# unibas-gravis/GiNGR

Hardware: AMD Instinct MI355X
Metric: GiNGR update iters/sec, 50k<->50k CPD (higher is better)
Workload: dtype f64; 1 GPU; CPD update, synthetic Gaussian clouds 50000<->50000, GPMM rank 100, w=0.1, rigid global transform, sigma2_0=5032.781; points=50000, targets=50000, rank=100, parallelism=row-shard x1, exchange=single shard

## Files before the change

gingr_amd/csrc/cpd_pairs.hip:

```cpp
#include "common.h"
#include "block_sum.h"
#include "box_device.h"
#include "cpd_plan.h"
#include "fastexp.h"

namespace {

constexpr int kBlock = 256;

constexpr int kTB = 11;
constexpr int kTabN = 1 << kTB;

#ifdef GINGR_STAMPS
__device__ unsigned long long *g_stamp_buf = nullptr;
constexpr int kStampWaves = 1 << 15;
struct Stamps {
    unsigned long long *p;
    long long c0;
    __device__ __forceinline__ void begin(int kernel) {
        const unsigned wg = blockIdx.y * gridDim.x + blockIdx.x;
        const unsigned w = wg * 4 + (threadIdx.x >> 6);
        p = (g_stamp_buf && w < kStampWaves) ? g_stamp_buf + ((size_t)kernel * kStampWaves + w) * 8 : nullptr;
        c0 = clock64();
        mark(0);
// ... 83 lines not shown
    unsigned long long act, slot[PT];
    const double *sub;
    const int32_t *bad;
    double negc;

    __device__ __forceinline__ void init(int64_t c0_, int64_t c1_, int q_, const double *sub_, const int32_t *bad_, double negc_) {
        c0 = c0_;
        c1 = c1_;
        q = q_;
        sub = sub_;
        bad = bad_;
        negc = negc_;
        t0 = c0 / kTile;
        nparts = c1 > c0 ? (int)((c1 - 1) / kTile - t0 + 1) : 0;
        pbase = 0;
        act = 0;
    }
    __device__ __forceinline__ void bounds(int p, int64_t *ib, int64_t *ie) const {
        const int64_t a = (t0 + p) * kTile, b = a + kTile;
        *ib = a > c0 ? a : c0;
        *ie = b < c1 ? b : c1;
    }
    __device__ __forceinline__ void batch(const Box &own, const Box (&sown)[PT]) {
        const int lane = threadIdx.x & 63;
        const int p = pbase + lane;
        int64_t ib, ie;
        bounds(p, &ib, &ie);
        const bool has = p < nparts && q * 64 < (int)(ie - ib);
        bool on = has;
        bool son[PT];
#pragma unroll
        for (int t = 0; t < PT; ++t) son[t] = has;
        if (has && sub && !(bad && bad[(t0 + p)])) {
            const double *qbox = sub + (ib / 64 + q) * 6;
            if (FINE) {
                on = false;
#pragma unroll
                for (int t = 0; t < PT; ++t) {
                    son[t] = !(box_gap2(sown[t], qbox) * negc > GINGR_CULL_SCALED(kTabN));
                    on = on || son[t];
                }
            } else {
                on = !(box_gap2(own, qbox) * negc > GINGR_CULL_SCALED(kTabN));
            }
        }
        act = __ballot(on);
        if (FINE) {
#pragma unroll
            for (int t = 0; t < PT; ++t) slot[t] = __ballot(son[t]);
        }
        pbase += 64;
    }
    __device__ __forceinline__ bool next(const Box &own, const Box (&sown)[PT], int64_t *ib, int64_t *ie, unsigned *mask) {
        while (act == 0) {
            if (pbase >= nparts) return false;
            batch(own, sown);
        }
        const int l = __builtin_ctzll(act);
        act &= act - 1;
        bounds(pbase - 64 + l, ib, ie);
        unsigned m = (1u << PT) - 1u;
        if (FINE) {
            m = 0;
#pragma unroll
            for (int t = 0; t < PT; ++t) m |= (unsigned)((slot[t] >> l) & 1ull) << t;
        }
        *mask = m;
        return true;
    }
};

__device__ __forceinline__ void fair_priority(int64_t done, int64_t total) {
    const int64_t f = total > 0 ? (4 * done) / total : 3;
    if (f <= 0)
        __builtin_amdgcn_s_setprio(3);
    else if (f == 1)
        __builtin_amdgcn_s_setprio(2);
    else if (f == 2)
        __builtin_amdgcn_s_setprio(1);
    else
        __builtin_amdgcn_s_setprio(0);
}

template <int PT, bool CLAMP, bool MASKED>
__device__ __forceinline__ void colsum_tile(const P4 *tile, int j0, int j1, unsigned mask, const double (&x)[PT],
                                            const double (&y)[PT], const double (&z)[PT], double (&acc)[PT], double c, double lim,
                                            const double *T) {
#pragma unroll 2
    for (int ii = j0; ii < j1; ++ii) {
        const P4 p = tile[ii];
#pragma unroll
        for (int t = 0; t < PT; ++t) {
            if (MASKED && !((mask >> t) & 1u)) continue;
            const double dx = x[t] - p.x, dy = y[t] - p.y, dz = z[t] - p.z;
            double d2 = __builtin_fma(dz, dz, __builtin_fma(dy, dy, dx * dx));
            if (CLAMP) d2 = fastexp_clamp_d2(d2, lim);
            acc[t] += fastexp2_floor_scaled(d2, c, T);
        }
    }
}

constexpr double kExpandTol = 1e-12;

__device__ __forceinline__ bool use_expansion(double rmax_centered, double c) {
    const double ratio = 3.0 * rmax_centered * rmax_centered * (-c) * (0.69314718055994530942 / kTabN);
    return ratio * 7.7e-16 < kExpandTol;
}

__device__ __forceinline__ double expand_owned_magic(double n, double *frac) {
    const double ni = __builtin_rint(n);
    *frac = n - ni;
    return GINGR_EXP_MAGIC8 + ni;
}
__device__ __forceinline__ double expand_owned_scale(double frac) { return exp2(frac * (1.0 / kTabN)); }

template <int PT, bool MASKED>
__device__ __forceinline__ void colsum_tile_expand(const P4 *tile, int j0, int j1, unsigned mask, const double (&x)[PT],
                                                   const double (&y)[PT], const double (&z)[PT], const double (&mg)[PT],
                                                   double (&acc)[PT], const double *T) {
#pragma unroll 2
    for (int ii = j0; ii < j1; ++ii) {
        const P4 p = tile[ii];
#pragma unroll
        for (int t = 0; t < PT; ++t) {
            if (MASKED && !((mask >> t) & 1u)) continue;
            const double A = __builtin_fma(z[t], p.z, __builtin_fma(y[t], p.y, __builtin_fma(x[t], p.x, p.w)));
            acc[t] += fastexp2_floor_core(A + mg[t], __builtin_amdgcn_fract(A), T);
        }
    }
}

template <int PT, bool FINE>
__global__ __launch_bounds__(kBlock) void cpd_colsum_kernel(Cloud fit, Cloud tgt, const double *__restrict__ sigma2,
                                                            const double *__restrict__ aux,
                                                            const double *__restrict__ fit_boxes, ChunkPlan plan,
                                                            double *__restrict__ partial, int32_t *regime_out) {
    __shared__ double T[kTabN];
    __shared__ P4 tile[kTile];
    __shared__ double sred[4][64 * PT];
    __shared__ double sfrac[64 * PT];
    STAMP_DECL
    STAMP_BEGIN(0)
    FloorTableRegs trom;
    fastexp_floor_table_fetch256(trom);
    const double s2in = sigma2[0], aux0 = aux[0], aux1 = aux[1], cx = aux[2], cy = aux[3], cz = aux[4];
    const int tid = threadIdx.x, lane = tid & 63;
    const int q = __builtin_amdgcn_readfirstlane(tid >> 6);
    const int64_t jbase = (int64_t)blockIdx.x * (64 * PT) + lane;
    double x[PT], y[PT], z[PT], n[PT], acc[PT];
    bool okv[PT];
#pragma unroll
    for (int t = 0; t < PT; ++t) {
        const int64_t j = jbase + (int64_t)t * 64;
        const bool ok = j < tgt.n;
        okv[t] = ok;
        x[t] = ok ? tgt.x[j] : 0.0;
        y[t] = ok ? tgt.y[j] : 0.0;
        z[t] = ok ? tgt.z[j] : 0.0;
    }
    int64_t i0, i1;
    plan.range(blockIdx.y, fit.n, &i0, &i1);
    const int q0 = q * 64;
    double lx = 0.0, ly = 0.0, lz = 0.0;
    const int64_t spec_ib = i0;
    {
        const int64_t e = min((i0 / kTile + 1) * kTile, i1), i = i0 + q0 + lane;
        if (i < e) {
            lx = fit.x[i];
            ly = fit.y[i];
            lz = fit.z[i];
        }
    }
    const double c = fastexp_scale_for_variance<kTB>(2.0 * s2in);
    const double am = aux0 + aux1;
    if (regime_out && blockIdx.x == 0 && blockIdx.y == 0 && threadIdx.x == 0) {
        *regime_out = (fit_boxes && 3.0 * am * am * (-c) > kFineCullRatio * GINGR_CULL_SCALED(kTabN)) ? 1 : 0;
        __threadfence_system();
    }
    const bool clamp = fastexp_needs_clamp(3.0 * am * am, c);
    const bool expand = use_expansion(fmax(aux0, aux1), c);
    const double lim = fastexp_d2_limit<kTB>(c);
    const double m2c = -2.0 * c;
    fastexp_floor_table_park256(T, trom);
    const Box own = wave_bbox<PT>(x, y, z, okv);
    constexpr unsigned kAllSlots = (1u << PT) - 1u;
    Box sown[PT];
    if (FINE) slot_boxes<PT>(x, y, z, okv, sown);
    const double *fit_sub = fit_boxes ? fit_boxes + ((fit.n + kTile - 1) / kTile) * 6 : nullptr;
#pragma unroll
    for (int t = 0; t < PT; ++t) {
        if (expand) {
            x[t] -= cx;
            y[t] -= cy;
            z[t] -= cz;
        }
        double fr;
        n[t] = expand_owned_magic(c * __builtin_fma(z[t], z[t], __builtin_fma(y[t], y[t], x[t] * x[t])), &fr);
        if (q == 0) sfrac[t * 64 + lane] = fr;
        acc[t] = 0.0;
    }
    STAMP(1)
    __syncthreads();
    STAMP(2)
    fastexp_round_down();
    struct Work {
        int64_t ib, ie;
        unsigned mask;
        bool valid;
    };
    PartWalk<PT, FINE> walk;
    walk.init(i0, i1, q, fit_boxes ? fit_sub : nullptr, nullptr, -c);
    auto find = [&]() {
        Work w{0, 0, kAllSlots, false};
        w.valid = walk.next(own, sown, &w.ib, &w.ie, &w.mask);
        return w;
    };
    auto issue = [&](const Work &w) {
        const int64_t i = w.ib + q0 + lane;
        if (i < w.ie) {
            lx = fit.x[i];
            ly = fit.y[i];
            lz = fit.z[i];
        }
    };
    Work cur = find();
    if (cur.valid && cur.ib != spec_ib) issue(cur);
#ifdef GINGR_STAMPS
    bool first__ = true;
#endif
    while (cur.valid) {
        if (plan.fair) fair_priority(cur.ib - i0, i1 - i0);
        __builtin_amdgcn_wave_barrier();
        if (cur.ib + q0 + lane < cur.ie) {
            if (expand) {
                const double fx = lx - cx, fy = ly - cy, fz = lz - cz;
                tile[q0 + lane] = P4{m2c * fx, m2c * fy, m2c * fz, c * __builtin_fma(fz, fz, __builtin_fma(fy, fy, fx * fx))};
            } else {
                tile[q0 + lane] = P4{lx, ly, lz, 0.0};
            }
        }
        __builtin_amdgcn_wave_barrier();
#ifdef GINGR_STAMPS
        if (first__) { STAMP(3) first__ = false; }
#endif
        const Work nxt = find();
        if (nxt.valid) issue(nxt);
        const int q1 = min((int)(cur.ie - cur.ib), q0 + 64);
        const unsigned mask = cur.mask;
        if (expand) {
            if (!FINE || mask == kAllSlots)
                colsum_tile_expand<PT, false>(tile, q0, q1, mask, x, y, z, n, acc, T);
            else
                colsum_tile_expand<PT, true>(tile, q0, q1, mask, x, y, z, n, acc, T);
        } else if (clamp) {
            if (!FINE || mask == kAllSlots)
                colsum_tile<PT, true, false>(tile, q0, q1, mask, x, y, z, acc, c, lim, T);
            else
                colsum_tile<PT, true, true>(tile, q0, q1, mask, x, y, z, acc, c, lim, T);
        } else {
            if (!FINE || mask == kAllSlots)
                colsum_tile<PT, false, false>(tile, q0, q1, mask, x, y, z, acc, c, lim, T);
            else
                colsum_tile<PT, false, true>(tile, q0, q1, mask, x, y, z, acc, c, lim, T);
        }
        cur = nxt;
    }
    fastexp_round_nearest();
    STAMP(4)
#pragma unroll
    for (int t = 0; t < PT; ++t) sred[q][t * 64 + lane] = acc[t];
    __syncthreads();
    for (int p = tid; p < 64 * PT; p += kBlock) {
        double v = (sred[0][p] + sred[1][p]) + (sred[2][p] + sred[3][p]);
        if (expand) v *= expand_owned_scale(sfrac[p]);
        const int64_t j = (int64_t)blockIdx.x * (64 * PT) + p;
        if (j < tgt.n) partial[(int64_t)blockIdx.y * tgt.n + j] = v;
    }
    STAMP_END
}

__global__ void chunk_reduce_kernel(const double *__restrict__ partial, int nchunks, int64_t n, double *__restrict__ out) {
    const int64_t j = (int64_t)blockIdx.x * blockDim.x + threadIdx.x;
    if (j >= n) return;
    double s = 0.0;
    for (int c = 0; c < nchunks; ++c) s += partial[(int64_t)c * n + j];
    out[j] = s;
}

constexpr int kScalarBlocks = 256;

__global__ __launch_bounds__(256) void cpd_den_finalize_kernel(Cloud tgt, const double *__restrict__ sigma2, double w,
                                                               double m_over_n, double *__restrict__ den,
                                                               double *__restrict__ inv_den, double *__restrict__ Pt1,
                                                               int32_t *__restrict__ tile_bad, double *__restrict__ part,
                                                               double *__restrict__ scalars,
                                                               const double *__restrict__ chunk_partial, int nchunks) {
    __shared__ double sh[256];
    const double s2 = sigma2[0];
    const double c = w / (1.0 - w) * pow(2.0 * 3.14159265358979323846 * s2, 1.5) * m_over_n;
    double xpx = 0.0;
    for (int64_t jt = (int64_t)blockIdx.x * 256; jt < tgt.n; jt += (int64_t)kScalarBlocks * 256) {
        const int64_t j = jt + threadIdx.x;
        int bad = 0;
        if (j < tgt.n) {
        double colsum;
        if (chunk_partial) {
            colsum = 0.0;
#pragma unroll 8
            for (int ch = 0; ch < nchunks; ++ch) colsum += chunk_partial[(int64_t)ch * tgt.n + j];
        } else {
            colsum = den[j];
        }
        const double d = colsum + c;
        const double inv = 1.0 / d;
        const double pt1 = colsum / d;
        den[j] = d;
        inv_den[j] = inv;
        Pt1[j] = pt1;
        bad = !(fabs(inv) <= 1.79769313486231570815e308);
        const double xx = tgt.x[j], yy = tgt.y[j], zz = tgt.z[j];
        xpx += pt1 * (xx * xx + yy * yy + zz * zz);
        }
        const int any_bad = __syncthreads_or(bad);
        if (tile_bad && threadIdx.x == 0) tile_bad[jt / kTile] = any_bad;
    }
    const double tot = block_sum<256>(xpx, sh);
    if (threadIdx.x == 0) {
        part[blockIdx.x] = tot;
        if (blockIdx.x == 0) scalars[5] = c;
    }
}

template <int PT, bool CLAMP, bool MASKED>
__device__ __forceinline__ void rowstats_tile(const P4 *tile, const P4 *tw, int j0, int j1, unsigned mask,
                                              const double (&x)[PT], const double (&y)[PT], const double (&z)[PT],
                                              double (&a1)[PT], double (&ax)[PT], double (&ay)[PT], double (&az)[PT], double c,
                                              double lim, const double *T) {
#pragma unroll 2
    for (int jj = j0; jj < j1; ++jj) {
        const P4 p = tile[jj];
        const P4 q = tw[jj];
#pragma unroll
        for (int t = 0; t < PT; ++t) {
            if (MASKED && !((mask >> t) & 1u)) continue;
            const double dx = p.x - x[t], dy = p.y - y[t], dz = p.z - z[t];
            double d2 = __builtin_fma(dz, dz, __builtin_fma(dy, dy, dx * dx));
            if (CLAMP) d2 = fastexp_clamp_d2(d2, lim);
            const double k = fastexp2_floor_scaled(d2, c, T);
            a1[t] = __builtin_fma(k, p.w, a1[t]);
            ax[t] = __builtin_fma(k, q.x, ax[t]);
            ay[t] = __builtin_fma(k, q.y, ay[t]);
            az[t] = __builtin_fma(k, q.z, az[t]);
        }
    }
}

template <int PT, bool MASKED>
__device__ __forceinline__ void rowstats_tile_expand(const P4 *tile, const P4 *tw, int j0, int j1, unsigned mask,
                                                     const double (&x)[PT], const double (&y)[PT], const double (&z)[PT],
                                                     const double (&mg)[PT], double (&a1)[PT], double (&ax)[PT], double (&ay)[PT],
                                                     double (&az)[PT], const double *T) {
#pragma unroll 2
    for (int jj = j0; jj < j1; ++jj) {
        const P4 p = tile[jj];
        const P4 q = tw[jj];
#pragma unroll
        for (int t = 0; t < PT; ++t) {
            if (MASKED && !((mask >> t) & 1u)) continue;
            const double A = __builtin_fma(z[t], p.z, __builtin_fma(y[t], p.y, __builtin_fma(x[t], p.x, p.w)));
            const double k = fastexp2_floor_core(A + mg[t], __builtin_amdgcn_fract(A), T);
            a1[t] = __builtin_fma(k, q.w, a1[t]);
            ax[t] = __builtin_fma(k, q.x, ax[t]);
            ay[t] = __builtin_fma(k, q.y, ay[t]);
            az[t] = __builtin_fma(k, q.z, az[t]);
        }
    }
}

template <int PT, bool FINE>
__global__ __launch_bounds__(kBlock, (PT >= 4 ? 3 : 4)) void cpd_rowstats_kernel(Cloud fit, Cloud tgt, const double *__restrict__ sigma2,
                                                              const double *__restrict__ aux,
                                                              const double *__restrict__ inv_den,
                                                              const double *__restrict__ tgt_boxes,
                                                              const int32_t *__restrict__ tile_bad, ChunkPlan plan,
                                                              double *__restrict__ partial, int32_t *regime_out) {
    constexpr int kRed = 4 * 4 * 64 * PT;
    constexpr int kLoop = kTabN + 4 * kTile + 4 * kTile;
    __shared__ double smem[kRed > kLoop ? kRed : kLoop];
    __shared__ double sfrac[64 * PT];
    double *T = smem;
    P4 *tile = reinterpret_cast<P4 *>(smem + kTabN);
    P4 *tw = reinterpret_cast<P4 *>(smem + kTabN + 4 * kTile);
    STAMP_DECL
    STAMP_BEGIN(1)
    FloorTableRegs trom;
    fastexp_floor_table_fetch256(trom);
    const double s2in = sigma2[0], aux0 = aux[0], aux1 = aux[1], cx = aux[2], cy = aux[3], cz = aux[4];
    const int tid = threadIdx.x, lane = tid & 63;
    const int q = __builtin_amdgcn_readfirstlane(tid >> 6);
    const int64_t ibase = (int64_t)blockIdx.x * (64 * PT) + lane;
    double x[PT], y[PT], z[PT], n[PT], a1[PT], ax[PT], ay[PT], az[PT];
    bool okv[PT];
#pragma unroll
    for (int t = 0; t < PT; ++t) {
        const int64_t i = ibase + (int64_t)t * 64;
        const bool ok = i < fit.n;
        okv[t] = ok;
        x[t] = ok ? fit.x[i] : 0.0;
        y[t] = ok ? fit.y[i] : 0.0;
        z[t] = ok ? fit.z[i] : 0.0;
    }
    int64_t j0, j1;
    plan.range(blockIdx.y, tgt.n, &j0, &j1);
    const int q0 = q * 64;
    double lx = 0.0, ly = 0.0, lz = 0.0, linv = 0.0;
    const int64_t spec_jb = j0;
    {
        const int64_t e = min((j0 / kTile + 1) * kTile, j1), j = j0 + q0 + lane;
        if (j < e) {
            lx = tgt.x[j];
            ly = tgt.y[j];
            lz = tgt.z[j];
            linv = inv_den[j];
        }
    }
    const double c = fastexp_scale_for_variance<kTB>(2.0 * s2in);
    const double am = aux0 + aux1;
    if (regime_out && blockIdx.x == 0 && blockIdx.y == 0 && threadIdx.x == 0) {
        *regime_out = (tgt_boxes && 3.0 * am * am * (-c) > kFineCullRatio * GINGR_CULL_SCALED(kTabN)) ? 1 : 0;
        __threadfence_system();
    }
    const bool clamp = fastexp_needs_clamp(3.0 * am * am, c);
    const bool expand = use_expansion(fmax(aux0, aux1), c);
    const double lim = fastexp_d2_limit<kTB>(c);
    const double m2c = -2.0 * c;
    fastexp_floor_table_park256(T, trom);
    const Box own = wave_bbox<PT>(x, y, z, okv);
    constexpr unsigned kAllSlots = (1u << PT) - 1u;
    Box sown[PT];
    if (FINE) slot_boxes<PT>(x, y, z, okv, sown);
    const double *tgt_sub = tgt_boxes ? tgt_boxes + ((tgt.n + kTile - 1) / kTile) * 6 : nullptr;
#pragma unroll
    for (int t = 0; t < PT; ++t) {
        if (expand) {
            x[t] -= cx;
            y[t] -= cy;
            z[t] -= cz;
        }
        double fr;
        n[t] = expand_owned_magic(c * __builtin_fma(z[t], z[t], __builtin_fma(y[t], y[t], x[t] * x[t])), &fr);
        if (q == 0) sfrac[t * 64 + lane] = fr;
        a1[t] = ax[t] = ay[t] = az[t] = 0.0;
    }
    STAMP(1)
    __syncthreads();
    STAMP(2)
    fastexp_round_down();
    struct Work {
        int64_t jb, je;
        unsigned mask;
        bool valid;
    };
    PartWalk<PT, FINE> walk;
    walk.init(j0, j1, q, tgt_boxes ? tgt_sub : nullptr, tgt_boxes ? tile_bad : nullptr, -c);
    auto find = [&]() {
        Work w{0, 0, kAllSlots, false};
        w.valid = walk.next(own, sown, &w.jb, &w.je, &w.mask);
        return w;
    };
    auto issue = [&](const Work &w) {
        const int64_t j = w.jb + q0 + lane;
        if (j < w.je) {
            lx = tgt.x[j];
            ly = tgt.y[j];
            lz = tgt.z[j];
            linv = inv_den[j];
        }
    };
    Work cur = find();
    if (cur.valid && cur.jb != spec_jb) issue(cur);
#ifdef GINGR_STAMPS
    bool first__ = true;
#endif
    while (cur.valid) {
        if (plan.fair) fair_priority(cur.jb - j0, j1 - j0);
        __builtin_amdgcn_wave_barrier();
        if (cur.jb + q0 + lane < cur.je) {
            const double inv = linv;
            if (expand) {
                const double tx = lx - cx, ty = ly - cy, tz = lz - cz;
                const double ax_ = m2c * tx, ay_ = m2c * ty, az_ = m2c * tz;
                tile[q0 + lane] = P4{ax_, ay_, az_, c * __builtin_fma(tz, tz, __builtin_fma(ty, ty, tx * tx))};
                tw[q0 + lane] = P4{ax_ * inv, ay_ * inv, az_ * inv, inv};
            } else {
                tile[q0 + lane] = P4{lx, ly, lz, inv};
                tw[q0 + lane] = P4{lx * inv, ly * inv, lz * inv, inv};
            }
        }
        __builtin_amdgcn_wave_barrier();
#ifdef GINGR_STAMPS
        if (first__) { STAMP(3) first__ = false; }
#endif
        const Work nxt = find();
        if (nxt.valid) issue(nxt);
        const int q1 = min((int)(cur.je - cur.jb), q0 + 64);
        const unsigned mask = cur.mask;
        if (expand) {
            if (!FINE || mask == kAllSlots)
                rowstats_tile_expand<PT, false>(tile, tw, q0, q1, mask, x, y, z, n, a1, ax, ay, az, T);
            else
                rowstats_tile_expand<PT, true>(tile, tw, q0, q1, mask, x, y, z, n, a1, ax, ay, az, T);
        } else if (clamp) {
            if (!FINE || mask == kAllSlots)
                rowstats_tile<PT, true, false>(tile, tw, q0, q1, mask, x, y, z, a1, ax, ay, az, c, lim, T);
            else
                rowstats_tile<PT, true, true>(tile, tw, q0, q1, mask, x, y, z, a1, ax, ay, az, c, lim, T);
        } else {
            if (!FINE || mask == kAllSlots)
                rowstats_tile<PT, false, false>(tile, tw, q0, q1, mask, x, y, z, a1, ax, ay, az, c, lim, T);
            else
                rowstats_tile<PT, false, true>(tile, tw, q0, q1, mask, x, y, z, a1, ax, ay, az, c, lim, T);
        }
        cur = nxt;
    }
    fastexp_round_nearest();
    STAMP(4)
    __syncthreads();
    constexpr int kPts = 64 * PT;
    double *sred = smem;
#pragma unroll
    for (int t = 0; t < PT; ++t) {
        sred[(q * 4 + 0) * kPts + t * 64 + lane] = a1[t];
        sred[(q * 4 + 1) * kPts + t * 64 + lane] = ax[t];
        sred[(q * 4 + 2) * kPts + t * 64 + lane] = ay[t];
        sred[(q * 4 + 3) * kPts + t * 64 + lane] = az[t];
    }
    __syncthreads();
    const int64_t M = fit.n;
    double *base = partial + (int64_t)blockIdx.y * 4 * M;
    const double back = expand ? -0.5 / c : 1.0;
    for (int p = tid; p < kPts; p += kBlock) {
        double v[4];
#pragma unroll
        for (int pl = 0; pl < 4; ++pl)
            v[pl] = (sred[(0 * 4 + pl) * kPts + p] + sred[(1 * 4 + pl) * kPts + p]) + (sred[(2 * 4 + pl) * kPts + p] + sred[(3 * 4 + pl) * kPts + p]);
        if (expand) {
            const double e = expand_owned_scale(sfrac[p]);
#pragma unroll
            for (int pl = 0; pl < 4; ++pl) v[pl] *= e;
        }
        const int64_t i = (int64_t)blockIdx.x * kPts + p;
        if (i < M) {
            base[i] = v[0];
            base[M + i] = expand ? __builtin_fma(cx, v[0], back * v[1]) : v[1];
            base[2 * M + i] = expand ? __builtin_fma(cy, v[0], back * v[2]) : v[2];
            base[3 * M + i] = expand ? __builtin_fma(cz, v[0], back * v[3]) : v[3];
        }
    }
    STAMP_END
}

template <int ROWS>
__global__ __launch_bounds__(4 * ROWS) void rowstats_reduce_kernel(const double *__restrict__ partial, int nchunks, Cloud fit,
                                                                   double *__restrict__ P1, double *__restrict__ PX,
                                                                   double *__restrict__ part, CpdObsArgs obs) {
    __shared__ double sh[ROWS];
    __shared__ double quart[3][4][ROWS];
    const int64_t M = fit.n;
    const int row = threadIdx.x % ROWS, g = threadIdx.x / ROWS;
    const int c0 = (int)((int64_t)g * nchunks / 4), c1 = (int)((int64_t)(g + 1) * nchunks / 4);
    double np = 0.0, tr = 0.0, ypy = 0.0;
    for (int64_t i0 = (int64_t)blockIdx.x * ROWS; i0 < M; i0 += (int64_t)kScalarBlocks * ROWS) {
        const int64_t i = i0 + row;
        const bool ok = i < M;
        double v[4] = {0.0, 0.0, 0.0, 0.0};
        double yx = 0.0, yy = 0.0, yz = 0.0, rf[3] = {0.0, 0.0, 0.0}, mn[3] = {0.0, 0.0, 0.0};
        int masked = 0;
        if (ok) {
            if (g == 0) {
                yx = fit.x[i];
                yy = fit.y[i];
                yz = fit.z[i];
                if (obs.weight) {
                    masked = obs.lm_mask ? obs.lm_mask[i] : 0;
#pragma unroll
                    for (int d = 0; d < 3; ++d) {
                        rf[d] = obs.ref[d * M + i];
                        mn[d] = obs.mean[d * M + i];
                    }
                }
            }
            const double *b = partial + i;
#pragma unroll 4
            for (int c = c0; c < c1; ++c) {
                const double *bc = b + (int64_t)c * 4 * M;
                v[0] += bc[0];
                v[1] += bc[M];
                v[2] += bc[2 * M];
                v[3] += bc[3 * M];
            }
        }
        if (g > 0) {
#pragma unroll
            for (int pl = 0; pl < 4; ++pl) quart[g - 1][pl][row] = v[pl];
        }
        __syncthreads();
        if (g == 0 && ok) {
#pragma unroll
            for (int pl = 0; pl < 4; ++pl) v[pl] = (v[pl] + quart[0][pl][row]) + (quart[1][pl][row] + quart[2][pl][row]);
            P1[i] = v[0];
            PX[i] = v[1];
            PX[M + i] = v[2];
            PX[2 * M + i] = v[3];
            if (obs.weight) {
                if (masked) {
                    obs.weight[i] = 0.0;
                    obs.evec[i] = obs.evec[M + i] = obs.evec[2 * M + i] = 0.0;
                } else {
                    const double p1inv = 1.0 / v[0];
                    const double ox = yx + (v[1] * p1inv - yx), oy = yy + (v[2] * p1inv - yy), oz = yz + (v[3] * p1inv - yz);
                    const double wgt = 1.0 / (obs.sigma2[0] * obs.lambda * p1inv);
                    const double *R = obs.R;
                    const double dx = ox - obs.center[0] - obs.t[0], dy = oy - obs.center[1] - obs.t[1], dz = oz - obs.center[2] - obs.t[2];
                    const double ex = R[0] * dx + R[3] * dy + R[6] * dz - (rf[0] - obs.center[0]) - mn[0];
                    const double ey = R[1] * dx + R[4] * dy + R[7] * dz - (rf[1] - obs.center[1]) - mn[1];
                    const double ez = R[2] * dx + R[5] * dy + R[8] * dz - (rf[2] - obs.center[2]) - mn[2];
                    obs.weight[i] = wgt;
                    obs.evec[i] = wgt * ex;
                    obs.evec[M + i] = wgt * ey;
                    obs.evec[2 * M + i] = wgt * ez;
                }
            }
            np += v[0];
            tr += yx * v[1] + yy * v[2] + yz * v[3];
            ypy += v[0] * (yx * yx + yy * yy + yz * yz);
        }
        __syncthreads();
    }
    double tot[3] = {0.0, 0.0, 0.0};
    const double vals[3] = {np, tr, ypy};
#pragma unroll
    for (int q = 0; q < 3; ++q) {
        if (g == 0) sh[row] = vals[q];
        __syncthreads();
#pragma unroll
        for (int st = ROWS / 2; st > 0; st >>= 1) {
            if (g == 0 && row < st) sh[row] += sh[row + st];
            __syncthreads();
        }
        tot[q] = sh[0];
        __syncthreads();
    }
    if (threadIdx.x == 0) {
        part[kScalarBlocks + blockIdx.x] = tot[0];
        part[2 * kScalarBlocks + blockIdx.x] = tot[1];
        part[3 * kScalarBlocks + blockIdx.x] = tot[2];
    }
}
__global__ __launch_bounds__(256) void cpd_scalars_finish_kernel(const double *__restrict__ part, double *__restrict__ scalars,
                                                                 double *__restrict__ xch8, int contribute_xpx) {
    __shared__ double sh[256];
    const int map[4] = {1, 0, 2, 3};
    for (int q = 0; q < 4; ++q) {
        const double tot = block_sum<256>(part[q * kScalarBlocks + threadIdx.x], sh);
        if (threadIdx.x == 0) {
            scalars[map[q]] = tot;
            if (xch8) xch8[map[q]] = (map[q] == 1 && !contribute_xpx) ? 0.0 : tot;
        }
        __syncthreads();
    }
    if (xch8 && threadIdx.x >= 4 && threadIdx.x < 8) xch8[threadIdx.x] = 0.0;
}

inline int resident_workgroups(int which ) {
    static int cache[3] = {0, 0, 0};
    if (cache[which] > 0) return cache[which];
    int per_cu = 0, dev = 0;
    hipError_t e;
    if (which == 0)
        e = hipOccupancyMaxActiveBlocksPerMultiprocessor(&per_cu, cpd_colsum_kernel<GINGR_PT_DEFAULT, false>, kBlock, 0);
    else if (which == 1)
        e = hipOccupancyMaxActiveBlocksPerMultiprocessor(&per_cu, cpd_rowstats_kernel<2, false>, kBlock, 0);
    else
        e = hipOccupancyMaxActiveBlocksPerMultiprocessor(&per_cu, cpd_rowstats_kernel<GINGR_PT_DEFAULT, false>, kBlock, 0);
    if (e != hipSuccess || per_cu < 1) per_cu = which == 2 ? 3 : 4;
    hipDeviceProp_t prop;
    int cus = 256;
    if (hipGetDevice(&dev) == hipSuccess && hipGetDeviceProperties(&prop, dev) == hipSuccess && prop.multiProcessorCount > 0)
        cus = prop.multiProcessorCount;
    (void)hipGetLastError();
    cache[which] = per_cu * cus;
    return cache[which];
}

constexpr int64_t kFineMinStream = 24576;

inline bool fine_variant(const gingr_ctx *ctx, const double *boxes, int64_t stream_len) {
    return boxes && (ctx->fine_override >= 0 ? ctx->fine_override != 0
                                             : (stream_len >= kFineMinStream && ctx->regime_host &&
                                                *(volatile int32_t *)ctx->regime_host != 0));
}

inline int colsum_resident() { return resident_workgroups(0); }
inline int rowstats_resident(int64_t M, int64_t N) { return resident_workgroups(rowstats_pt(M, N) == 2 ? 1 : 2); }

}

int64_t cpd_colsum_ws_doubles(int64_t M, int64_t N) { return colsum_ws_doubles(M, N, colsum_resident()); }
int cpd_colsum_chunks(int64_t M, int64_t N) { return colsum_plan(M, N, 0, colsum_resident()).nch; }
int64_t cpd_rowstats_ws_doubles(int64_t M, int64_t N) { return rowstats_ws_doubles(M, N, rowstats_resident(M, N)); }

int launch_cpd_colsum(gingr_ctx *ctx, Cloud fit, Cloud target, const double *sigma2_dev, const double *aux,
                      const double *fit_boxes, double *ws, double *den_partial, int forced_chunks) {
    const PairPlan pp = colsum_plan(fit.n, target.n, forced_chunks, colsum_resident());
    {
        TimerScope ts(ctx, 0);
        dim3 grid((unsigned)ceil_div(target.n, 64 * pp.pt), (unsigned)pp.nch);
        const double *boxes = ctx->cull ? fit_boxes : (const double *)nullptr;
        const bool fine = fine_variant(ctx, boxes, fit.n);
        int32_t *regime_out = boxes ? ctx->regime_dev : (int32_t *)nullptr;
        auto launch = [&](auto kern) {
            hipLaunchKernelGGL(kern, grid, dim3(kBlock), 0, ctx->stream, fit, target, sigma2_dev, aux, boxes, pp.plan, ws, regime_out);
        };
        if (pp.pt == 1)
            launch(cpd_colsum_kernel<1, false>);
        else if (pp.pt == 2)
            launch(cpd_colsum_kernel<2, false>);
        else if (fine)
            launch(cpd_colsum_kernel<kPT, true>);
        else
            launch(cpd_colsum_kernel<kPT, false>);
    }
    if (den_partial)
        hipLaunchKernelGGL(chunk_reduce_kernel, dim3((unsigned)ceil_div(target.n, 256)), dim3(256), 0, ctx->stream, ws, pp.nch,
                           target.n, den_partial);
    return pp.nch;
}

void launch_cpd_den_finalize(gingr_ctx *ctx, Cloud target, const double *sigma2_dev, double w, int64_t M_total,
                             double *den, double *inv_den, double *Pt1, int32_t *tile_bad, double *part,
                             double *scalars_dev, const double *chunk_partial, int nchunks) {
    hipLaunchKernelGGL(cpd_den_finalize_kernel, dim3(kScalarBlocks), dim3(256), 0, ctx->stream, target, sigma2_dev, w,
                       (double)M_total / (double)target.n, den, inv_den, Pt1, tile_bad, part, scalars_dev, chunk_partial, nchunks);
}

void launch_cpd_rowstats(gingr_ctx *ctx, Cloud fit, Cloud target, const double *sigma2_dev, const double *aux,
                         const double *inv_den, const double *tgt_boxes, const int32_t *tile_bad, double *ws, double *P1,
                         double *PX_soa, double *part, double *scalars_dev, double *xch8, int contribute_xpx,
                         const CpdObsArgs *obs, bool finish_scalars) {
    const PairPlan pp = rowstats_plan(fit.n, target.n, rowstats_resident(fit.n, target.n));
    {
        TimerScope ts(ctx, 1);
        dim3 grid((unsigned)ceil_div(fit.n, 64 * pp.pt), (unsigned)pp.nch);
        const bool cull = ctx->cull && tgt_boxes && tile_bad;
        const double *boxes = cull ? tgt_boxes : (const double *)nullptr;
        const bool fine = fine_variant(ctx, boxes, target.n);
        int32_t *regime_out = boxes ? ctx->regime_dev : (int32_t *)nullptr;
        auto launch = [&](auto kern) {
            hipLaunchKernelGGL(kern, grid, dim3(kBlock), 0, ctx->stream, fit, target, sigma2_dev, aux, inv_den, boxes, tile_bad,
                               pp.plan, ws, regime_out);
        };
        if (pp.pt == 1) {
            launch(cpd_rowstats_kernel<1, false>);
        } else if (pp.pt == 2) {
            if (fine)
                launch(cpd_rowstats_kernel<2, true>);
            else
                launch(cpd_rowstats_kernel<2, false>);
// ... 38 lines not shown
```

gingr_amd/csrc/cpd_plan.h:

```cpp
#pragma once
#include <cstdint>

#include "host_device.h"

constexpr int kTile = 256;
constexpr int kNNThreads = 64;

struct ChunkPlan {
    int64_t len_big, len_tail;
    int32_t n_big;
    int32_t fair = 0;
    GINGR_HD void range(int64_t y, int64_t n, int64_t *b, int64_t *e) const {
        const int64_t lo = y < n_big ? y * len_big : (int64_t)n_big * len_big + (y - n_big) * len_tail;
        const int64_t hi = lo + (y < n_big ? len_big : len_tail);
        *b = lo;
        *e = hi < n ? hi : n;
    }
    int chunks(int64_t n) const {
        const int64_t head = (int64_t)n_big * len_big;
        if (head >= n) return (int)((n + len_big - 1) / len_big);
        return n_big + (int)((n - head + len_tail - 1) / len_tail);
    }
};

#ifndef GINGR_PT
#define GINGR_PT 4
#endif
#define GINGR_PT_DEFAULT GINGR_PT
constexpr int kPT = GINGR_PT_DEFAULT;
#ifndef GINGR_SMALL_COLSUM_COLS
#define GINGR_SMALL_COLSUM_COLS 16384
#endif
#ifndef GINGR_SMALL_SHARD_ROWS
#define GINGR_SMALL_SHARD_ROWS 2048
#endif
constexpr int64_t kSmallShardRows = GINGR_SMALL_SHARD_ROWS;
constexpr int64_t kSmallColsumCols = GINGR_SMALL_COLSUM_COLS;
constexpr int64_t kTinyCols = 2048;
#ifndef GINGR_ROWSTATS_PT
#define GINGR_ROWSTATS_PT 0
#endif
#ifndef GINGR_COLSUM_QUARTERS
#define GINGR_COLSUM_QUARTERS 0
#endif
#ifndef GINGR_ROWSTATS_QUARTERS
#define GINGR_ROWSTATS_QUARTERS 0
#endif
#ifndef GINGR_COLSUM_CHUNKS
#define GINGR_COLSUM_CHUNKS 0
#endif
#ifndef GINGR_ROWSTATS_CHUNKS
#define GINGR_ROWSTATS_CHUNKS 0
#endif
#ifndef GINGR_FAIR_PRIORITY
#define GINGR_FAIR_PRIORITY 1
#endif
#ifndef GINGR_COLSUM_PT
#define GINGR_COLSUM_PT 0
#endif
inline int colsum_pt(int64_t cols) {
    constexpr int forced = GINGR_COLSUM_PT;
    if (forced == 1 || forced == 2 || forced == kPT) return forced;
    if (kPT > 2 && cols <= kTinyCols) return 1;
    return (kPT > 2 && cols <= kSmallColsumCols) ? 2 : kPT;
}
inline int rowstats_pt(int64_t rows, int64_t cols) {
    constexpr int forced = GINGR_ROWSTATS_PT;
    if (forced == 1 || forced == 2 || forced == kPT) return forced;
    if (kPT > 2 && rows <= kTinyCols && cols <= kTinyCols) return 1;
    return (kPT > 2 && (rows <= kSmallShardRows || (rows <= kSmallColsumCols && cols <= kSmallColsumCols))) ? 2 : kPT;
}
constexpr int kTargetBlocks = 5120;
#ifndef GINGR_MIN_CHUNK
#define GINGR_MIN_CHUNK 256
#endif
constexpr int kMinChunk = GINGR_MIN_CHUNK;

inline ChunkPlan plan_chunks(int64_t owned, int owned_per_block, int64_t stream_len, int *nchunks, int quarters_override = 0,
                             int forced_chunks = 0, int resident = 0) {
    const int64_t bx = ceil_div(owned, owned_per_block);
    int64_t want = ceil_div(kTargetBlocks, bx > 0 ? bx : 1);
    if (want < 1) want = 1;
    const int64_t n = stream_len > 0 ? stream_len : 1;
    int64_t len = round_up(ceil_div(n, want), 64);
    if (quarters_override > 0) len = (int64_t)quarters_override * 64;
    if (len >= kTile)
        len = round_up(len, kTile);
    else if (len > 128)
        len = kTile;
    else if (len > 64)
        len = 128;
    else
        len = 64;
    if (quarters_override <= 0 && len < kMinChunk) len = kMinChunk;
    ChunkPlan p{len, len, (int32_t)ceil_div(n, len), 0};
    int forced = forced_chunks;
    if (forced <= 0 && quarters_override <= 0 && resident > 0) {
        int64_t k = (kTargetBlocks + resident / 2) / resident;
        const int64_t kmax = (n / 1024) * (bx > 0 ? bx : 1) / resident;
        if (k > kmax) k = kmax;
        if (k < 1) k = 1;
        int64_t nc = k * resident / (bx > 0 ? bx : 1);
        const int64_t Qmax = ceil_div(n, 64);
        if (nc > Qmax) nc = Qmax;
        if (nc < 1) nc = 1;
        if (Qmax / nc >= 16) forced = (int)nc;
    }
    if (forced > 0) {
        const int64_t Q = ceil_div(n, 64), q = Q / forced, rem = Q % forced;
        if (q >= 1) {
            p.len_big = (q + 1) * 64;
            p.len_tail = q * 64;
            p.n_big = (int32_t)rem;
            if (rem == 0) {
                p.len_big = p.len_tail;
                p.n_big = forced;
            }
        }
    }
    *nchunks = p.chunks(n);
    constexpr int fair_env = GINGR_FAIR_PRIORITY;
    p.fair = (fair_env == 2 || (fair_env == 1 && resident > 0 && (int64_t)*nchunks * bx <= resident)) ? 1 : 0;
    return p;
// ... 47 lines not shown
```

gingr_amd/csrc/fastexp.h:

```cpp
#pragma once

#include <hip/hip_runtime.h>

#define GINGR_EXP_TABLE 2048
#define GINGR_EXP_TABLE_LOG2 11
#define GINGR_EXP_MAGIC 6755399441055744.0

template <int TB>
struct ExpTab;
template <>
struct ExpTab<11> {
    static constexpr double C1 = 3.38450771757785784e-04;
    static constexpr double C2 = 5.72744624517204032e-08;
    static constexpr double C3 = 6.46152867293236500e-12;
    static constexpr double C1_D2 = 3.384507729693224e-04;
};
__device__ static const double gingr_exp_table_rom[2048] = {
#include "exp_table.inc"
};
template <int TB = 11>
__device__ __forceinline__ void fastexp_table_init(double *T) {
    static_assert(TB == 11, "one table size");
    const double *rom = gingr_exp_table_rom;
    for (int j = threadIdx.x + threadIdx.y * blockDim.x; j < (1 << TB); j += blockDim.x * blockDim.y) T[j] = rom[j];
}

template <int DEG = 3, int TB = 11>
__device__ __forceinline__ double fastexp2_core(double tm, double f, const double *T) {
    const unsigned long long bits = __builtin_bit_cast(unsigned long long, tm);
    const unsigned lo = (unsigned)bits, hi = (unsigned)(bits >> 32);
    const int e = (int)__builtin_amdgcn_alignbit(hi, lo, TB);
    double q;
    if (DEG == 3) {
        q = __builtin_fma(f, ExpTab<TB>::C3, ExpTab<TB>::C2);
        q = __builtin_fma(f, q, ExpTab<TB>::C1);
    } else {
        q = __builtin_fma(f, ExpTab<TB>::C2, ExpTab<TB>::C1_D2);
    }
    const double tj = T[lo & ((1u << TB) - 1)];
    const double fq = f * q;
    const double r = __builtin_fma(tj, fq, tj);
    return __builtin_ldexp(r, e);
}

template <int DEG = 3, int TB = 11>
__device__ __forceinline__ double fastexp2_scaled(double d2, double c, const double *T) {
    const double tm = __builtin_fma(d2, c, GINGR_EXP_MAGIC);
    const double kf = tm - GINGR_EXP_MAGIC;
    const double f = __builtin_fma(d2, c, -kf);
    return fastexp2_core<DEG, TB>(tm, f, T);
}

struct ExpFloor11 {
    static constexpr double Q0 = 3.384507681227659e-04;
    static constexpr double Q1 = 5.728415556485551e-08;
    static constexpr double S = 0x1.000000000038dp+0;
};

__device__ __forceinline__ void fastexp_round_down() { asm volatile("s_setreg_imm32_b32 hwreg(HW_REG_MODE, 2, 2), 2\n\ts_nop 3" ::: "memory"); }
__device__ __forceinline__ void fastexp_round_nearest() { asm volatile("s_setreg_imm32_b32 hwreg(HW_REG_MODE, 2, 2), 0\n\ts_nop 3" ::: "memory"); }

__device__ static const double gingr_exp_floor_table_rom[2048] __attribute__((aligned(16))) = {
#include "exp_floor_table.inc"
};
typedef double fastexp_v2f64 __attribute__((ext_vector_type(2)));
struct FloorTableRegs {
    fastexp_v2f64 v0, v1, v2, v3;
};
__device__ __forceinline__ void fastexp_floor_table_fetch256(FloorTableRegs &r) {
    const fastexp_v2f64 *rom = reinterpret_cast<const fastexp_v2f64 *>(gingr_exp_floor_table_rom) + threadIdx.x;
    r.v0 = rom[0];
    r.v1 = rom[256];
    r.v2 = rom[512];
    r.v3 = rom[768];
}
__device__ __forceinline__ void fastexp_floor_table_park256(double *T, const FloorTableRegs &r) {
    fastexp_v2f64 *t2 = reinterpret_cast<fastexp_v2f64 *>(T) + threadIdx.x;
    t2[0] = r.v0;
    t2[256] = r.v1;
    t2[512] = r.v2;
    t2[768] = r.v3;
}

#define GINGR_EXP_MAGIC8 844424930131968.0

__device__ __forceinline__ double fastexp2_floor_core(double tm, double f, const double *T) {
    const unsigned long long bits = __builtin_bit_cast(unsigned long long, tm);
    const unsigned lo = (unsigned)bits, hi = (unsigned)(bits >> 32);
    const int e = (int)__builtin_amdgcn_alignbit(hi, lo, 14);
    const double q = __builtin_fma(f, ExpFloor11::Q1, ExpFloor11::Q0);
    const double tj = *reinterpret_cast<const double *>(reinterpret_cast<const char *>(T) + (lo & 0x3FF8u));
    const double fq = f * q;
    const double r = __builtin_fma(tj, fq, tj);
    return __builtin_ldexp(r, e);
}

__device__ __forceinline__ double fastexp2_floor_scaled(double d2, double c, const double *T) {
    const double u = d2 * c;
    return fastexp2_floor_core(u + GINGR_EXP_MAGIC8, __builtin_amdgcn_fract(u), T);
}

template <int TB = 11>
__device__ __forceinline__ double fastexp_scale_for_variance(double two_sigma2) {
    return -(double)(1 << TB) * 1.4426950408889634074 / two_sigma2;
}

template <int TB = 11>
__device__ __forceinline__ double fastexp_d2_limit(double c) {
    return -1100.0 * (double)(1 << TB) / c;
}

__device__ __forceinline__ double fastexp_clamp_d2(double d2, double lim) {
    const double m = fmin(d2, lim);
    return d2 == d2 ? m : d2;
}

__device__ __forceinline__ bool fastexp_needs_clamp(double d2_bound, double c) {
    return !(d2_bound * (-c) < 2199023255552.0);
}
```

Baseline: 459.3 iterations/s.

## Interleave rowstats tile pairs in LDS and hand-schedule tile loops with fixed-address reader

Stores the rowstats tile and weight tile interleaved in one LDS array so each pair is read with two adjacent 16-byte loads per entry, via a TileReader that keeps a single incrementing LDS address register. Replaces the unroll-2 loops with a macro loop that unrolls by 4 with a sched_barrier for PT>=4, and hoists the polynomial constant Q0 into a VGPR through an opaque asm so it is not rematerialised per call. It also changes the non-FINE rowstats launch bound to a configurable wave count, defaulting to 4 instead of 3, which may raise occupancy but increase register pressure or spilling.

Result: no change. 461.7 iterations/s, median of 6 (+0.5%).

```diff
diff --git a/gingr_amd/csrc/cpd_pairs.hip b/gingr_amd/csrc/cpd_pairs.hip
--- a/gingr_amd/csrc/cpd_pairs.hip
+++ b/gingr_amd/csrc/cpd_pairs.hip
@@ -189,22 +189,64 @@
         __builtin_amdgcn_s_setprio(0);
 }
 
+typedef double lds_v2f64 __attribute__((ext_vector_type(2)));
+template <int STRIDE>
+struct TileReader {
+    unsigned a;
+    __device__ __forceinline__ explicit TileReader(const P4 *first) {
+        a = (unsigned)(uintptr_t)(const __attribute__((address_space(3))) P4 *)first;
+        asm volatile("" : "+v"(a));
+    }
+    __device__ __forceinline__ P4 entry(int k, int plus = 0) const {
+        typedef const __attribute__((address_space(3))) lds_v2f64 *Ptr;
+        const unsigned off = 32u * (unsigned)(STRIDE * k + plus);
+        const lds_v2f64 lo = *(Ptr)(uintptr_t)(a + off), hi = *(Ptr)(uintptr_t)(a + (off + 16u));
+        return P4{lo.x, lo.y, hi.x, hi.y};
+    }
+    __device__ __forceinline__ void step(int n) { a += 32u * (unsigned)(STRIDE * n); }
+};
+#define GINGR_TILE_LOOP(FOUR, rd, j0, j1, load, pairs)                 \
+    {                                                                  \
+        int ii__ = (j0);                                               \
+        if (FOUR) {                                                    \
+            _Pragma("unroll 1") for (; ii__ + 4 <= (j1); ii__ += 4) {  \
+                pairs(load(0));                                        \
+                pairs(load(1));                                        \
+                __builtin_amdgcn_sched_barrier(0);                     \
+                pairs(load(2));                                        \
+                pairs(load(3));                                        \
+                (rd).step(4);                                          \
+            }                                                          \
+        } else {                                                       \
+            _Pragma("unroll 1") for (; ii__ + 2 <= (j1); ii__ += 2) {  \
+                pairs(load(0));                                        \
+                pairs(load(1));                                        \
+                (rd).step(2);                                          \
+            }                                                          \
+        }                                                              \
+        _Pragma("unroll 1") for (; ii__ < (j1); ++ii__) {              \
+            pairs(load(0));                                            \
+            (rd).step(1);                                              \
+        }                                                              \
+    }
+
 template <int PT, bool CLAMP, bool MASKED>
 __device__ __forceinline__ void colsum_tile(const P4 *tile, int j0, int j1, unsigned mask, const double (&x)[PT],
                                             const double (&y)[PT], const double (&z)[PT], double (&acc)[PT], double c, double lim,
-                                            const double *T) {
-#pragma unroll 2
-    for (int ii = j0; ii < j1; ++ii) {
-        const P4 p = tile[ii];
+                                            const double *T, double q0) {
+    TileReader<1> rd(tile + j0);
+    auto pairs = [&](const P4 p) __attribute__((always_inline)) {
 #pragma unroll
         for (int t = 0; t < PT; ++t) {
             if (MASKED && !((mask >> t) & 1u)) continue;
             const double dx = x[t] - p.x, dy = y[t] - p.y, dz = z[t] - p.z;
             double d2 = __builtin_fma(dz, dz, __builtin_fma(dy, dy, dx * dx));
             if (CLAMP) d2 = fastexp_clamp_d2(d2, lim);
-            acc[t] += fastexp2_floor_scaled(d2, c, T);
-        }
-    }
+            acc[t] += fastexp2_floor_scaled(d2, c, T, q0);
+        }
+    };
+    auto load = [&](int k) __attribute__((always_inline)) { return rd.entry(k); };
+    GINGR_TILE_LOOP(false, rd, j0, j1, load, pairs)
 }
 
 constexpr double kExpandTol = 1e-12;
@@ -224,17 +266,18 @@
 template <int PT, bool MASKED>
 __device__ __forceinline__ void colsum_tile_expand(const P4 *tile, int j0, int j1, unsigned mask, const double (&x)[PT],
                                                    const double (&y)[PT], const double (&z)[PT], const double (&mg)[PT],
-                                                   double (&acc)[PT], const double *T) {
-#pragma unroll 2
-    for (int ii = j0; ii < j1; ++ii) {
-        const P4 p = tile[ii];
+                                                   double (&acc)[PT], const double *T, double q0) {
+    TileReader<1> rd(tile + j0);
+    auto pairs = [&](const P4 p) __attribute__((always_inline)) {
 #pragma unroll
         for (int t = 0; t < PT; ++t) {
             if (MASKED && !((mask >> t) & 1u)) continue;
             const double A = __builtin_fma(z[t], p.z, __builtin_fma(y[t], p.y, __builtin_fma(x[t], p.x, p.w)));
-            acc[t] += fastexp2_floor_core(A + mg[t], __builtin_amdgcn_fract(A), T);
-        }
-    }
+            acc[t] += fastexp2_floor_core(A + mg[t], __builtin_amdgcn_fract(A), T, q0);
+        }
+    };
+    auto load = [&](int k) __attribute__((always_inline)) { return rd.entry(k); };
+    GINGR_TILE_LOOP(false, rd, j0, j1, load, pairs)
 }
 
 template <int PT, bool FINE>
@@ -288,6 +331,7 @@
     const bool expand = use_expansion(fmax(aux0, aux1), c);
     const double lim = fastexp_d2_limit<kTB>(c);
     const double m2c = -2.0 * c;
+    const double expq0 = fastexp_floor_q0();
     fastexp_floor_table_park256(T, trom);
     const Box own = wave_bbox<PT>(x, y, z, okv);
     constexpr unsigned kAllSlots = (1u << PT) - 1u;
@@ -356,19 +400,19 @@
         const unsigned mask = cur.mask;
         if (expand) {
             if (!FINE || mask == kAllSlots)
-                colsum_tile_expand<PT, false>(tile, q0, q1, mask, x, y, z, n, acc, T);
+                colsum_tile_expand<PT, false>(tile, q0, q1, mask, x, y, z, n, acc, T, expq0);
             else
-                colsum_tile_expand<PT, true>(tile, q0, q1, mask, x, y, z, n, acc, T);
+                colsum_tile_expand<PT, true>(tile, q0, q1, mask, x, y, z, n, acc, T, expq0);
         } else if (clamp) {
             if (!FINE || mask == kAllSlots)
-                colsum_tile<PT, true, false>(tile, q0, q1, mask, x, y, z, acc, c, lim, T);
+                colsum_tile<PT, true, false>(tile, q0, q1, mask, x, y, z, acc, c, lim, T, expq0);
             else
-                colsum_tile<PT, true, true>(tile, q0, q1, mask, x, y, z, acc, c, lim, T);
+                colsum_tile<PT, true, true>(tile, q0, q1, mask, x, y, z, acc, c, lim, T, expq0);
         } else {
             if (!FINE || mask == kAllSlots)
-                colsum_tile<PT, false, false>(tile, q0, q1, mask, x, y, z, acc, c, lim, T);
+                colsum_tile<PT, false, false>(tile, q0, q1, mask, x, y, z, acc, c, lim, T, expq0);
             else
-                colsum_tile<PT, false, true>(tile, q0, q1, mask, x, y, z, acc, c, lim, T);
+                colsum_tile<PT, false, true>(tile, q0, q1, mask, x, y, z, acc, c, lim, T, expq0);
         }
         cur = nxt;
     }
@@ -438,54 +482,59 @@
     }
 }
 
+struct TilePair {
+    P4 p, q;
+};
 template <int PT, bool CLAMP, bool MASKED>
-__device__ __forceinline__ void rowstats_tile(const P4 *tile, const P4 *tw, int j0, int j1, unsigned mask,
+__device__ __forceinline__ void rowstats_tile(const P4 *tile, int j0, int j1, unsigned mask,
                                               const double (&x)[PT], const double (&y)[PT], const double (&z)[PT],
                                               double (&a1)[PT], double (&ax)[PT], double (&ay)[PT], double (&az)[PT], double c,
-                                              double lim, const double *T) {
-#pragma unroll 2
-    for (int jj = j0; jj < j1; ++jj) {
-        const P4 p = tile[jj];
-        const P4 q = tw[jj];
+                                              double lim, const double *T, double q0) {
+    TileReader<2> rd(tile + 2 * j0);
+    auto pairs = [&](const TilePair e) __attribute__((always_inline)) {
+        const P4 p = e.p, q = e.q;
 #pragma unroll
         for (int t = 0; t < PT; ++t) {
             if (MASKED && !((mask >> t) & 1u)) continue;
             const double dx = p.x - x[t], dy = p.y - y[t], dz = p.z - z[t];
             double d2 = __builtin_fma(dz, dz, __builtin_fma(dy, dy, dx * dx));
             if (CLAMP) d2 = fastexp_clamp_d2(d2, lim);
-            const double k = fastexp2_floor_scaled(d2, c, T);
+            const double k = fastexp2_floor_scaled(d2, c, T, q0);
             a1[t] = __builtin_fma(k, p.w, a1[t]);
             ax[t] = __builtin_fma(k, q.x, ax[t]);
             ay[t] = __builtin_fma(k, q.y, ay[t]);
             az[t] = __builtin_fma(k, q.z, az[t]);
         }
-    }
+    };
+    auto load = [&](int k) __attribute__((always_inline)) { return TilePair{rd.entry(k), rd.entry(k, 1)}; };
+    GINGR_TILE_LOOP(PT >= 4, rd, j0, j1, load, pairs)
 }
 
 template <int PT, bool MASKED>
-__device__ __forceinline__ void rowstats_tile_expand(const P4 *tile, const P4 *tw, int j0, int j1, unsigned mask,
+__device__ __forceinline__ void rowstats_tile_expand(const P4 *tile, int j0, int j1, unsigned mask,
                                                      const double (&x)[PT], const double (&y)[PT], const double (&z)[PT],
                                                      const double (&mg)[PT], double (&a1)[PT], double (&ax)[PT], double (&ay)[PT],
-                                                     double (&az)[PT], const double *T) {
-#pragma unroll 2
-    for (int jj = j0; jj < j1; ++jj) {
-        const P4 p = tile[jj];
-        const P4 q = tw[jj];
+                                                     double (&az)[PT], const double *T, double q0) {
+    TileReader<2> rd(tile + 2 * j0);
+    auto pairs = [&](const TilePair e) __attribute__((always_inline)) {
+        const P4 p = e.p, q = e.q;
 #pragma unroll
         for (int t = 0; t < PT; ++t) {
             if (MASKED && !((mask >> t) & 1u)) continue;
             const double A = __builtin_fma(z[t], p.z, __builtin_fma(y[t], p.y, __builtin_fma(x[t], p.x, p.w)));
-            const double k = fastexp2_floor_core(A + mg[t], __builtin_amdgcn_fract(A), T);
+            const double k = fastexp2_floor_core(A + mg[t], __builtin_amdgcn_fract(A), T, q0);
             a1[t] = __builtin_fma(k, q.w, a1[t]);
             ax[t] = __builtin_fma(k, q.x, ax[t]);
             ay[t] = __builtin_fma(k, q.y, ay[t]);
             az[t] = __builtin_fma(k, q.z, az[t]);
         }
-    }
+    };
+    auto load = [&](int k) __attribute__((always_inline)) { return TilePair{rd.entry(k), rd.entry(k, 1)}; };
+    GINGR_TILE_LOOP(PT >= 4, rd, j0, j1, load, pairs)
 }
 
 template <int PT, bool FINE>
-__global__ __launch_bounds__(kBlock, (PT >= 4 ? 3 : 4)) void cpd_rowstats_kernel(Cloud fit, Cloud tgt, const double *__restrict__ sigma2,
+__global__ __launch_bounds__(kBlock, (PT >= 4 ? (FINE ? 3 : GINGR_ROWSTATS_WAVES) : 4)) void cpd_rowstats_kernel(Cloud fit, Cloud tgt, const double *__restrict__ sigma2,
                                                               const double *__restrict__ aux,
                                                               const double *__restrict__ inv_den,
                                                               const double *__restrict__ tgt_boxes,
@@ -497,7 +546,6 @@
     __shared__ double sfrac[64 * PT];
     double *T = smem;
     P4 *tile = reinterpret_cast<P4 *>(smem + kTabN);
-    P4 *tw = reinterpret_cast<P4 *>(smem + kTabN + 4 * kTile);
     STAMP_DECL
     STAMP_BEGIN(1)
     FloorTableRegs trom;
@@ -541,6 +589,7 @@
     const bool expand = use_expansion(fmax(aux0, aux1), c);
     const double lim = fastexp_d2_limit<kTB>(c);
     const double m2c = -2.0 * c;
+    const double expq0 = fastexp_floor_q0();
     fastexp_floor_table_park256(T, trom);
     const Box own = wave_bbox<PT>(x, y, z, okv);
     constexpr unsigned kAllSlots = (1u << PT) - 1u;
@@ -597,11 +646,11 @@
             if (expand) {
                 const double tx = lx - cx, ty = ly - cy, tz = lz - cz;
                 const double ax_ = m2c * tx, ay_ = m2c * ty, az_ = m2c * tz;
-                tile[q0 + lane] = P4{ax_, ay_, az_, c * __builtin_fma(tz, tz, __builtin_fma(ty, ty, tx * tx))};
-                tw[q0 + lane] = P4{ax_ * inv, ay_ * inv, az_ * inv, inv};
+                tile[2 * (q0 + lane)] = P4{ax_, ay_, az_, c * __builtin_fma(tz, tz, __builtin_fma(ty, ty, tx * tx))};
+                tile[2 * (q0 + lane) + 1] = P4{ax_ * inv, ay_ * inv, az_ * inv, inv};
             } else {
-                tile[q0 + lane] = P4{lx, ly, lz, inv};
-                tw[q0 + lane] = P4{lx * inv, ly * inv, lz * inv, inv};
+                tile[2 * (q0 + lane)] = P4{lx, ly, lz, inv};
+                tile[2 * (q0 + lane) + 1] = P4{lx * inv, ly * inv, lz * inv, inv};
             }
         }
         __builtin_amdgcn_wave_barrier();
@@ -614,19 +663,19 @@
         const unsigned mask = cur.mask;
         if (expand) {
             if (!FINE || mask == kAllSlots)
-                rowstats_tile_expand<PT, false>(tile, tw, q0, q1, mask, x, y, z, n, a1, ax, ay, az, T);
+                rowstats_tile_expand<PT, false>(tile, q0, q1, mask, x, y, z, n, a1, ax, ay, az, T, expq0);
             else
-                rowstats_tile_expand<PT, true>(tile, tw, q0, q1, mask, x, y, z, n, a1, ax, ay, az, T);
+                rowstats_tile_expand<PT, true>(tile, q0, q1, mask, x, y, z, n, a1, ax, ay, az, T, expq0);
         } else if (clamp) {
             if (!FINE || mask == kAllSlots)
-                rowstats_tile<PT, true, false>(tile, tw, q0, q1, mask, x, y, z, a1, ax, ay, az, c, lim, T);
+                rowstats_tile<PT, true, false>(tile, q0, q1, mask, x, y, z, a1, ax, ay, az, c, lim, T, expq0);
             else
-                rowstats_tile<PT, true, true>(tile, tw, q0, q1, mask, x, y, z, a1, ax, ay, az, c, lim, T);
+                rowstats_tile<PT, true, true>(tile, q0, q1, mask, x, y, z, a1, ax, ay, az, c, lim, T, expq0);
         } else {
             if (!FINE || mask == kAllSlots)
-                rowstats_tile<PT, false, false>(tile, tw, q0, q1, mask, x, y, z, a1, ax, ay, az, c, lim, T);
+                rowstats_tile<PT, false, false>(tile, q0, q1, mask, x, y, z, a1, ax, ay, az, c, lim, T, expq0);
             else
-                rowstats_tile<PT, false, true>(tile, tw, q0, q1, mask, x, y, z, a1, ax, ay, az, c, lim, T);
+                rowstats_tile<PT, false, true>(tile, q0, q1, mask, x, y, z, a1, ax, ay, az, c, lim, T, expq0);
         }
         cur = nxt;
     }
@@ -790,7 +839,8 @@
         e = hipOccupancyMaxActiveBlocksPerMultiprocessor(&per_cu, cpd_rowstats_kernel<2, false>, kBlock, 0);
     else
         e = hipOccupancyMaxActiveBlocksPerMultiprocessor(&per_cu, cpd_rowstats_kernel<GINGR_PT_DEFAULT, false>, kBlock, 0);
-    if (e != hipSuccess || per_cu < 1) per_cu = which == 2 ? 3 : 4;
+    if (e != hipSuccess || per_cu < 1) per_cu = which == 2 ? GINGR_ROWSTATS_WAVES : 4;
+    if (which == 2 && GINGR_ROWSTATS_PLAN_WAVES > 0) per_cu = GINGR_ROWSTATS_PLAN_WAVES;
     hipDeviceProp_t prop;
     int cus = 256;
     if (hipGetDevice(&dev) == hipSuccess && hipGetDeviceProperties(&prop, dev) == hipSuccess && prop.multiProcessorCount > 0)
diff --git a/gingr_amd/csrc/cpd_plan.h b/gingr_amd/csrc/cpd_plan.h
--- a/gingr_amd/csrc/cpd_plan.h
+++ b/gingr_amd/csrc/cpd_plan.h
@@ -39,6 +39,13 @@
 constexpr int64_t kTinyCols = 2048;
 #ifndef GINGR_ROWSTATS_PT
 #define GINGR_ROWSTATS_PT 0
+#endif
+#ifndef GINGR_ROWSTATS_WAVES
+#define GINGR_ROWSTATS_WAVES 4
+#endif
+static_assert(GINGR_ROWSTATS_WAVES == 3 || GINGR_ROWSTATS_WAVES == 4, "GINGR_ROWSTATS_WAVES: 3 or 4");
+#ifndef GINGR_ROWSTATS_PLAN_WAVES
+#define GINGR_ROWSTATS_PLAN_WAVES 0
 #endif
 #ifndef GINGR_COLSUM_QUARTERS
 #define GINGR_COLSUM_QUARTERS 0
diff --git a/gingr_amd/csrc/fastexp.h b/gingr_amd/csrc/fastexp.h
--- a/gingr_amd/csrc/fastexp.h
+++ b/gingr_amd/csrc/fastexp.h
@@ -84,20 +84,25 @@
 
 #define GINGR_EXP_MAGIC8 844424930131968.0
 
-__device__ __forceinline__ double fastexp2_floor_core(double tm, double f, const double *T) {
+__device__ __forceinline__ double fastexp_floor_q0() {
+    double q0 = ExpFloor11::Q0;
+    asm volatile("" : "+v"(q0));
+    return q0;
+}
+__device__ __forceinline__ double fastexp2_floor_core(double tm, double f, const double *T, double q0) {
     const unsigned long long bits = __builtin_bit_cast(unsigned long long, tm);
     const unsigned lo = (unsigned)bits, hi = (unsigned)(bits >> 32);
     const int e = (int)__builtin_amdgcn_alignbit(hi, lo, 14);
-    const double q = __builtin_fma(f, ExpFloor11::Q1, ExpFloor11::Q0);
+    const double q = __builtin_fma(f, ExpFloor11::Q1, q0);
     const double tj = *reinterpret_cast<const double *>(reinterpret_cast<const char *>(T) + (lo & 0x3FF8u));
     const double fq = f * q;
     const double r = __builtin_fma(tj, fq, tj);
     return __builtin_ldexp(r, e);
 }
 
-__device__ __forceinline__ double fastexp2_floor_scaled(double d2, double c, const double *T) {
+__device__ __forceinline__ double fastexp2_floor_scaled(double d2, double c, const double *T, double q0) {
     const double u = d2 * c;
-    return fastexp2_floor_core(u + GINGR_EXP_MAGIC8, __builtin_amdgcn_fract(u), T);
+    return fastexp2_floor_core(u + GINGR_EXP_MAGIC8, __builtin_amdgcn_fract(u), T, q0);
 }
 
 template <int TB = 11>
```
